# proroklab/gnn_pathplanning

Hardware: AMD Instinct MI355X
Metric: agent-steps/sec (policy fwd) (higher is better)
Workload: dtype f32 (bf16x3 exact operand split, f32 accumulate); 1 GPU; policy forward (addGSO+forward), 10 agents, 20x20 map GSO, K=3, batch=512 per GPU, eval mode, fp32 GSO resident in HBM; the SAME resident batch every step (inputs are L2 / Infinity-Cache warm by construction); agents=10, taps=3, batch_per_gpu=512, global_batch=512, parallelism=replicas x1

## Files before the change

### gnn_pathplanning_amd/csrc/encoder_kernel_b3.hip

```cpp
#include <utility>

#include "gnnpp_common.h"

namespace gnnpp {

constexpr int kb_L1 = 0, kb_L2 = 54, kb_L3 = 108, kb_L4 = 162, kb_FC = 270, kb_END = 294;
constexpr int kb_FILT = kb_END;

constexpr int kB3Frag = 1024;
constexpr int kB3Region = 25 * 3 * kB3Frag;
constexpr int kB3Obs2 = kObsFloatsLds * 4;
constexpr int kB3L2out = 0, kB3L3out = 24 * kB3Frag, kB3L4out = 48 * kB3Frag;
constexpr int kB3Table = kB3Region;
constexpr int kB3TableBytes = EncLayout::kBssFloats * 4 + 16;
constexpr int kB3TableBytesFused = 5120;
constexpr int kB3SsmOff = 776 * 4;
constexpr size_t kB3Smem = kB3Region + kB3TableBytes;
constexpr size_t kB3SmemFused = kB3Region + kB3TableBytesFused;
static_assert(2 * kObsFloatsLds * 4 <= kB3Region && kB3SsmOff + 16 * 17 * 4 <= kB3TableBytesFused &&
              2 * kB3SmemFused <= (size_t)kLdsBytes, "b3 LDS map");
constexpr int kB3ZBytes = 16 * kZs * 4;
constexpr int kB3PRow = 3 * 256 + 32;
constexpr int kB3PBytes = 16 * kB3PRow;
constexpr int kB3POff = 2 * kB3ZBytes;
static_assert(kB3POff + kPolicyTapsMax * kB3PBytes + 4 * 16 * 8 * 4 <= kB3Region, "fused tail fits R");
constexpr size_t policy_sim_occ_bytes_b3() {
    return (size_t)kB3POff - 8 * kMaxAgents * sizeof(int) - kGsoSmemBytes;
}

struct WStreamB {
    const float* seg[6];
    int lane_bytes;
};

__device__ __forceinline__ const float* ring_item_ptr(const WStreamB& ws, int idx) {
    if (idx < kb_L2) return ws.seg[0] + (idx - kb_L1) * EncLayout::kHItem;
    if (idx < kb_L3) return ws.seg[1] + (idx - kb_L2) * EncLayout::kHItem;
    if (idx < kb_L4) return ws.seg[2] + (idx - kb_L3) * EncLayout::kHItem;
    if (idx < kb_FC) return ws.seg[3] + (idx - kb_L4) * EncLayout::kHItem;
    if (idx < kb_FILT) return ws.seg[4] + (idx - kb_FC) * EncLayout::kHItem;
    const int j = idx - kb_FILT, pl = j % 3, ml = (j / 3) & 1, kb = (j / 6) & 3, tap = j / 24;
    return ws.seg[5] + tap * (8 * 4 * 768) + ml * (4 * 768) + kb * 768 + pl * 256;
}

template <int IT, int NKB, int H, int W, int NMT, int NSLOT, class PosFn, bool PRELOAD, int CH = NSLOT>
__device__ __forceinline__ void b3_tap_mfma(const v4f* in, const v4f* Pin, const v8b (&A)[NMT][3],
                                            v4f (&acc)[NSLOT][NMT], int lane) {
    constexpr int kb = IT / 9, tap = IT % 9;
    constexpr int dy = tap / 3 - 1, dx = tap % 3 - 1;
#pragma unroll
    for (int j0 = 0; j0 < NSLOT; j0 += CH) {
        v8b B[CH][3];
#pragma unroll
        for (int jj = 0; jj < CH; ++jj) {
            const int j = j0 + jj;
            int y = 0, x = 0;
            const bool used = j < NSLOT && PosFn::get(j, y, x);
            const int iy = y + dy, ix = x + dx;
            if (used && iy >= 0 && iy < H && ix >= 0 && ix < W) {
                const int o = ((iy * W + ix) * NKB + kb) * 3;
#pragma unroll
                for (int p = 0; p < 3; ++p) B[jj][p] = as_b8(PRELOAD ? Pin[o + p] : in[(o + p) * 64 + lane]);
            }
        }
#pragma unroll
        for (int term = 0; term < kB3Terms; ++term) {
#pragma unroll
            for (int jj = 0; jj < CH; ++jj) {
                const int j = j0 + jj;
                int y = 0, x = 0;
                const bool used = j < NSLOT && PosFn::get(j, y, x);
                const int iy = y + dy, ix = x + dx;
                if (used && iy >= 0 && iy < H && ix >= 0 && ix < W) {
// ... 210 lines not shown
            const int wy = win / 5, wx = win - wy * 5;
            const unsigned* base = obsw + (2 * wy) * kPadHW + 2 * wx;
            v4f acc[4][2];
#pragma unroll
            for (int pp = 0; pp < 4; ++pp) {
                unsigned d1[8], d2[8];
#pragma unroll
                for (int e = 0; e < 8; ++e) {
                    d1[e] = base[aoff[e] + (pp >> 1) * kPadHW + (pp & 1)];
                    d2[e] = base[kObsFloatsLds + aoff[e] + (pp >> 1) * kPadHW + (pp & 1)];
                }
                unsigned bh[4], bm[4], bl[4];
#pragma unroll
                for (int w = 0; w < 4; ++w) {
                    bh[w] = __builtin_amdgcn_perm(d1[2 * w + 1], d1[2 * w], 0x05040100u);
                    bm[w] = __builtin_amdgcn_perm(d1[2 * w + 1], d1[2 * w], 0x07060302u);
                    bl[w] = __builtin_amdgcn_perm(d2[2 * w + 1], d2[2 * w], 0x05040100u);
                }
                const v4u bhv = {bh[0], bh[1], bh[2], bh[3]}, bmv = {bm[0], bm[1], bm[2], bm[3]},
                          blv = {bl[0], bl[1], bl[2], bl[3]};
                const v8b B[3] = {__builtin_bit_cast(v8b, bhv), __builtin_bit_cast(v8b, bmv),
                                  __builtin_bit_cast(v8b, blv)};
#pragma unroll
                for (int term = 0; term < kB3Terms; ++term)
#pragma unroll
                    for (int i = 0; i < 2; ++i)
                        acc[pp][i] = mfma16b(A0[i][b3_term_a(term)], B[b3_term_b(term)],
                                             term == 0 ? vzero() : acc[pp][i]);
            }
#pragma unroll
            for (int i = 0; i < 2; ++i) {
                v4f sc, sh;
                load_ss(sstab + EncLayout::kBssL0, 32, i, q, sc, sh);
                v4f r = vmax(vmax(acc[0][i], acc[1][i]), vmax(acc[2][i], acc[3][i]));
                r = vfma(r, sc, sh);
#pragma unroll
                for (int c = 0; c < 4; ++c) r[c] = b3_relu_clamp(r[c]);
                res[wi][i] = r;
            }
        }
    }
    __syncthreads();
#pragma unroll
    for (int wi = 0; wi < 7; ++wi) {
        const int win = wave + 4 * wi;
        if (win < 25) {
            v4f pl[3];
            b3_split8_clamped(res[wi][0], res[wi][1], pl);
            b3_store_window<CP>(smem, g, win, lane, pl);
        }
    }
}

template <bool ONE_PLANE, bool CP>
__device__ __forceinline__ void b3_l0_stream(const float* __restrict__ pk, const unsigned* obsw,
                                             const float* sstab, char* smem, const CpGeom& g,
                                             v4f (&res)[ONE_PLANE ? 3 : 5][2], int wave, int lane) {
    constexpr int DEPTH = ONE_PLANE ? 3 : 1;
    constexpr int NHELD = ONE_PLANE ? 3 : 5;
    static_assert((4 * NHELD) * 3 * kB3Frag >= (ONE_PLANE ? 1 : 2) * kObsFloatsLds * 4, "held windows cover the pixels");
    constexpr int NW = ONE_PLANE ? 8 : 16;
    const int a = lane & 15, q = lane >> 4;
    v8b A0[2][3];
#pragma unroll
    for (int i = 0; i < 2; ++i)
#pragma unroll
        for (int p = 0; p < 3; ++p)
            A0[i][p] = as_b8(*reinterpret_cast<const v4f*>(pk + EncLayout::kB0 + ((i * 3 + p) * 64 + lane) * 4));
    int aoff[8];
#pragma unroll
    for (int e = 0; e < 8; ++e)
        aoff[e] = a * kAgentStride + (q < 3 ? q * (kPadHW * kPadHW) + (e / 3) * kPadHW + e % 3
                                            : e < 3 ? e * (kPadHW * kPadHW) + 2 * kPadHW + 2 : 0);
    v4f sc[2], sh[2];
    load_ss(sstab + EncLayout::kBssL0, 32, 0, q, sc[0], sh[0]);
    load_ss(sstab + EncLayout::kBssL0, 32, 1, q, sc[1], sh[1]);
    unsigned d[DEPTH + 1][NW];
    v4f acc[2][2];
    v4f run[2];
    auto request = [&](unsigned (&dd)[NW], int P) {
        const int win = wave + 4 * (P >> 2), pp = P & 3;
        const int wy = win / 5, wx = win - wy * 5;
        const unsigned* base = obsw + (2 * wy + (pp >> 1)) * kPadHW + 2 * wx + (pp & 1);
#pragma unroll
        for (int e = 0; e < 8; ++e) {
            dd[e] = base[aoff[e]];
            if (!ONE_PLANE) dd[8 + e] = base[kObsFloatsLds + aoff[e]];
        }
    };
    auto compute = [&](const unsigned (&dd)[NW], v4f (&ac)[2]) {
        unsigned bh[4], bm[4], bl[4];
#pragma unroll
        for (int w = 0; w < 4; ++w) {
            bh[w] = __builtin_amdgcn_perm(dd[2 * w + 1], dd[2 * w], 0x05040100u);
            if (!ONE_PLANE) {
                bm[w] = __builtin_amdgcn_perm(dd[2 * w + 1], dd[2 * w], 0x07060302u);
                bl[w] = __builtin_amdgcn_perm(dd[8 + 2 * w + 1], dd[8 + 2 * w], 0x05040100u);
            }
        }
        const v4u bhv = {bh[0], bh[1], bh[2], bh[3]};
        const v8b Bh = __builtin_bit_cast(v8b, bhv);
        if (ONE_PLANE) {
#pragma unroll
            for (int p = 2; p >= 0; --p)
#pragma unroll
                for (int i = 0; i < 2; ++i) ac[i] = mfma16b(A0[i][p], Bh, p == 2 ? vzero() : ac[i]);
        } else {
            const v4u bmv = {bm[0], bm[1], bm[2], bm[3]}, blv = {bl[0], bl[1], bl[2], bl[3]};
            const v8b B[3] = {Bh, __builtin_bit_cast(v8b, bmv), __builtin_bit_cast(v8b, blv)};
#pragma unroll
            for (int term = 0; term < kB3Terms; ++term)
#pragma unroll
                for (int i = 0; i < 2; ++i)
                    ac[i] = mfma16b(A0[i][b3_term_a(term)], B[b3_term_b(term)], term == 0 ? vzero() : ac[i]);
        }
    };
    auto epilogue = [&](const v4f (&ac)[2], int P) {
#pragma unroll
        for (int i = 0; i < 2; ++i) {
            run[i] = (P & 3) == 0 ? ac[i] : vmax(run[i], ac[i]);
            if ((P & 3) == 3) {
                run[i] = vfma(run[i], sc[i], sh[i]);
#pragma unroll
                for (int c = 0; c < 4; ++c) run[i][c] = b3_relu_clamp(run[i][c]);
            }
        }
#if defined(__HIP_DEVICE_COMPILE__)
        asm volatile("" : "+v"(run[0]), "+v"(run[1]));
#endif
    };
    auto window_done = [&](auto wic) {
        constexpr int wi = decltype(wic)::value;
        if constexpr (wi < NHELD) {
            res[wi][0] = run[0];
            res[wi][1] = run[1];
        } else {
            const int win = wave + 4 * wi;
            v4f pl[3];
            b3_split8_clamped(run[0], run[1], pl);
            b3_store_window<CP>(smem, g, win, lane, pl);
        }
    };
    auto prologue = [&](auto p0c, auto p1c, auto kc) {
        constexpr int P = decltype(p0c)::value + decltype(kc)::value;
        if constexpr (P < decltype(p1c)::value) request(d[P % (DEPTH + 1)], P);
    };
    auto body = [&](auto p0c, auto p1c, auto kc) {
        constexpr int P0 = decltype(p0c)::value, P1 = decltype(p1c)::value, P = P0 + decltype(kc)::value;
        if constexpr (P + DEPTH < P1) request(d[(P + DEPTH) % (DEPTH + 1)], P + DEPTH);
        __builtin_amdgcn_sched_barrier(0);
        compute(d[P % (DEPTH + 1)], acc[P & 1]);
        if constexpr (P > P0) {
            epilogue(acc[(P - 1) & 1], P - 1);
            if constexpr (((P - 1) & 3) == 3) window_done(std::integral_constant<int, ((P - 1) >> 2)>{});
        }
        __builtin_amdgcn_sched_barrier(0);
        if constexpr (P == P1 - 1) {
            epilogue(acc[P & 1], P);
            window_done(std::integral_constant<int, (P >> 2)>{});
        }
    };
    auto stream = [&](auto p0c, auto p1c) {
        constexpr int N = decltype(p1c)::value - decltype(p0c)::value;
        auto pro = [&](auto... ks) { (prologue(p0c, p1c, ks), ...); };
        auto run_all = [&](auto... ks) { (body(p0c, p1c, ks), ...); };
        [&]<int... K>(std::integer_sequence<int, K...>) { pro(std::integral_constant<int, K>{}...); }(
            std::make_integer_sequence<int, DEPTH>{});
        [&]<int... K>(std::integer_sequence<int, K...>) { run_all(std::integral_constant<int, K>{}...); }(
            std::make_integer_sequence<int, N>{});
    };
    stream(std::integral_constant<int, 0>{}, std::integral_constant<int, 24>{});
    if (wave == 0) stream(std::integral_constant<int, 24>{}, std::integral_constant<int, 28>{});
}

__host__ __device__ __forceinline__ constexpr int cp_ring_item_at(int NA, int i, int s) {
    int first = -1, cnt = 0;
    for (int k = 0; k < 6; ++k)
        if (k * NA / 6 == i) { if (first < 0) first = k; ++cnt; }
    if (cnt == 0 || s % (6 / cnt) != 0 || s / (6 / cnt) >= cnt) return -1;
    return first + s / (6 / cnt);
}
template <class Load, class Hook>
__device__ __forceinline__ void cp_unit(const v8b (&A)[2][3], const v4f (&B)[3], v4f& c0, v4f& c1, Load&& load, Hook&& hook) {
#define GNNPP_CP_M(T, ACC, MI)                                                                          \
    ACC = mfma16b(A[MI][b3_term_a(T)], as_b8(B[b3_term_b(T)]), ACC);                                   \
    __builtin_amdgcn_sched_barrier(0);
#define GNNPP_CP_H(S)                                                                                   \
    hook(std::integral_constant<int, S>{});                                                             \
    __builtin_amdgcn_sched_barrier(0);
    GNNPP_CP_M(0, c0, 0)
    load(0);
    __builtin_amdgcn_sched_barrier(0);
    GNNPP_CP_M(0, c1, 1)
    load(1);
    __builtin_amdgcn_sched_barrier(0);
    GNNPP_CP_M(1, c0, 0)
    load(2);
    __builtin_amdgcn_sched_barrier(0);
    GNNPP_CP_M(1, c1, 1)
    GNNPP_CP_H(0)
    GNNPP_CP_M(2, c0, 0)
    GNNPP_CP_H(1)
    GNNPP_CP_M(2, c1, 1)
    GNNPP_CP_H(2)
// ... 289 lines not shown
        case 2: cp_layer2_main<END, 2>(ws, ring, smem, ln, pair, acc); break;
        case 3: cp_layer2_main<END, 3>(ws, ring, smem, ln, pair, acc); break;
        case 4: cp_layer2_main<END, 4>(ws, ring, smem, ln, pair, acc); break;
        case 5: cp_layer2_main<END, 5>(ws, ring, smem, ln, pair, acc); break;
        default: cp_layer2_main<END, 6>(ws, ring, smem, ln, pair, acc); break;
    }
    v4f sc[2], shf[2];
    load_ss(sstab + EncLayout::kBssL2, 64, 2 * mp, q, sc[0], shf[0]);
    load_ss(sstab + EncLayout::kBssL2, 64, 2 * mp + 1, q, sc[1], shf[1]);
    const bool hi2 = (p & 2) != 0, hi1 = (p & 1) != 0;
    float pooled[NT][2];
#pragma unroll
    for (int i = 0; i < NT; ++i) {
        pooled[i][0] = pooled[i][1] = 0.f;
        if (i < na) {
            const v4f v0 = vfma(acc[i][0], sc[0], shf[0]), v1 = vfma(acc[i][1], sc[1], shf[1]);
            v4f keep, send;
#pragma unroll
            for (int c = 0; c < 4; ++c) {
                keep[c] = hi2 ? v1[c] : v0[c];
                send[c] = hi2 ? v0[c] : v1[c];
            }
#pragma unroll
            for (int c = 0; c < 4; ++c) keep[c] = fmaxf(keep[c], quad_xor2(send[c]));
            const float k0 = hi1 ? keep[2] : keep[0], k1 = hi1 ? keep[3] : keep[1];
            const float s0 = hi1 ? keep[0] : keep[2], s1 = hi1 ? keep[1] : keep[3];
            pooled[i][0] = fmaxf(fmaxf(k0, quad_xor1(s0)), 0.f);
            pooled[i][1] = fmaxf(fmaxf(k1, quad_xor1(s1)), 0.f);
        }
    }
    __syncthreads();
#pragma unroll
    for (int i = 0; i < NT; ++i) {
        if (i < na) {
            const int n = pair + 2 * i;
            unsigned h, m, l;
            b3_split2(pooled[i][0], pooled[i][1], h, m, l);
            char* const dst = smem + kB3L2out + ((w * 2 + mp) * 3) * kB3Frag + (q * 16 + n) * 16 + p * 4;
            *reinterpret_cast<unsigned*>(dst) = h;
            *reinterpret_cast<unsigned*>(dst + kB3Frag) = m;
            *reinterpret_cast<unsigned*>(dst + 2 * kB3Frag) = l;
        }
    }
    if (j >= g.N) {
#pragma unroll
        for (int k = 0; k < 6; ++k)
            *reinterpret_cast<v4f*>(smem + kB3L2out + (wave + 4 * k) * kB3Frag + lane * 16) = vzero();
    }
}

template <bool FUSED, int KT, bool CP = false>
__global__ GNNPP_H2_VGPR_BUDGET __launch_bounds__(kThreads, 2) void encoder_kernel_b3(const float* __restrict__ obs,
                                                                 const float* __restrict__ pk,
                                                                 float* __restrict__ feat, int M, int stop,
                                                                 const PolicyTail pt) {
    constexpr int END = FUSED ? kb_FILT + 24 * KT : kb_END;
    extern __shared__ __attribute__((aligned(16))) char gnnpp_smem[];
    v4f* const R4 = reinterpret_cast<v4f*>(gnnpp_smem);
    unsigned* const obsw = reinterpret_cast<unsigned*>(gnnpp_smem);
    float* const sstab = reinterpret_cast<float*>(gnnpp_smem + kB3Table);
    unsigned* const planeflag = reinterpret_cast<unsigned*>(gnnpp_smem + kB3Table + EncLayout::kBssFloats * 4);
    const int tid = threadIdx.x;
    const int lane = tid & 63;
    const int wave = __builtin_amdgcn_readfirstlane(tid >> 6);
    const int a = lane & 15;
    const int q = lane >> 4;
    const int tile_agents = (FUSED || CP) ? pt.N : kTileAgents;
    const int agent0 = blockIdx.x * tile_agents;
    const int n_agents = FUSED ? pt.N : min(tile_agents, M - agent0);
    const CpGeom geom = cp_geom(CP ? n_agents : kTileAgents);
    GNNPP_STAMP(blockIdx.x, 11, tid == 0);

    WStreamB ws;
    ws.seg[0] = pk + EncLayout::kB1;
    ws.seg[1] = pk + EncLayout::kB2 + (wave & 1) * (54 * EncLayout::kHItem);
    ws.seg[2] = pk + EncLayout::kB3 + wave * (54 * EncLayout::kHItem);
    ws.seg[3] = pk + EncLayout::kB4 + wave * (108 * EncLayout::kHItem);
    ws.seg[4] = pk + EncLayout::kBfcw + wave * (24 * EncLayout::kHItem);
    ws.seg[5] = FUSED ? pt.filt_h2 + wave * (2 * 4 * 768) : pk;
    ws.lane_bytes = lane * 16;
    float ssv[3];
#pragma unroll
    for (int i = 0; i < 3; ++i)
        ssv[i] = pk[EncLayout::kBss + min(tid + i * kThreads, EncLayout::kBssFloats - 1)];
    float hcv[4] = {0.f, 0.f, 0.f, 0.f};
    float sval = 0.f;
    if (FUSED) {
#pragma unroll
        for (int i = 0; i < 4; ++i) {
            const int c = tid + i * kThreads;
            if (c < 640) hcv[i] = pt.act_w[c];
            else if (c < 768) hcv[i] = pt.gf_bias ? pt.gf_bias[c - 640] : 0.f;
            else if (c < 773) hcv[i] = pt.act_b[c - 768];
        }
        const int m = tid >> 4, n = tid & 15;
        if (m < pt.N && n < pt.N) {
            const size_t i = ((size_t)blockIdx.x * pt.N + m) * pt.N + n;
            sval = pt.s_is_f64 ? (float)reinterpret_cast<const double*>(pt.S)[i]
                               : reinterpret_cast<const float*>(pt.S)[i];
        }
    }
    v4f ring[kRingH];
#if defined(__HIP_DEVICE_COMPILE__)
    asm volatile("; weight ring lives in v[208:255]" ::: "v255");
#endif
#pragma unroll
    for (int i = 0; i < kRingH; ++i) h2_ring_load<END>(ws, ring, i);

    {
        constexpr int NV4 = (kTileAgents * kObsFloats + 3) / 4 + 1;
        constexpr int PER = (NV4 + kThreads - 1) / kThreads;
        const int valid = n_agents * kObsFloats;
        const float* src = obs + (size_t)agent0 * kObsFloats;
        const int shift = (int)((reinterpret_cast<uintptr_t>(src) >> 2) & 3);
        const float* src4 = src - shift;
        const long floats_left = (long)(M - agent0) * kObsFloats + shift;
        const bool head_ok = shift == 0 || agent0 > 0;
        v4f v[PER];
#pragma unroll
        for (int k = 0; k < PER; ++k) {
            const int idx = tid + k * kThreads;
            const int e0 = 4 * idx - shift;
            if (head_ok && 4L * idx + 4 <= floats_left && e0 < valid) {
                v[k] = *reinterpret_cast<const v4f*>(src4 + 4 * idx);
            } else {
#pragma unroll
                for (int c = 0; c < 4; ++c) v[k][c] = src[min(max(e0 + c, 0), valid - 1)];
            }
        }
        for (int i = tid; i < 2 * kObsFloatsLds / 4; i += kThreads) R4[i] = vzero();
        if (CP && tid < kCpRow / 16)
            *reinterpret_cast<v4f*>(gnnpp_smem + geom.l1in + geom.T1 * kCpRow + tid * 16) = vzero();
        unsigned residual = 0;
#pragma unroll
        for (int i = 0; i < 3; ++i)
            if (tid + i * kThreads < EncLayout::kBssFloats) sstab[tid + i * kThreads] = ssv[i];
        __syncthreads();
        const unsigned dump = 2 * kObsFloatsLds + lane;
#pragma unroll
        for (int k = 0; k < PER; ++k) {
            const int e0 = (tid + k * kThreads) * 4 - shift;
            const unsigned es = (unsigned)max(e0, 0);
            const unsigned ag = __umul24(es, 46223u) >> 24;
            const unsigned rem = es - __umul24(ag, (unsigned)kObsFloats);
            const unsigned ch = __umul24(rem, 543u) >> 16;
            const int r0 = (int)(rem - __umul24(ch, 121u)) + min(e0, 0);
            const unsigned base = __umul24(ag, (unsigned)kAgentStride) + __umul24(ch, (unsigned)(kPadHW * kPadHW)) + 13u;
            const unsigned wrapped = base + (ch == 2u ? (unsigned)(kAgentStride - 2 * kPadHW * kPadHW) : (unsigned)(kPadHW * kPadHW));
            unsigned w1[4], w2[4];
            const v4u vb = __builtin_bit_cast(v4u, v[k]);
            const bool inexact = ((vb[0] | vb[1] | vb[2] | vb[3]) & 0xffffu) != 0u;
            const bool any_l = __ballot(inexact) != 0ull;
            if (!any_l) {
                w1[0] = vb[0] >> 16; w1[1] = vb[1] >> 16; w1[2] = vb[2] >> 16; w1[3] = vb[3] >> 16;
            } else {
#pragma unroll
                for (int c2 = 0; c2 < 2; ++c2) {
                    unsigned h, m, l;
                    b3_split2(v[k][2 * c2], v[k][2 * c2 + 1], h, m, l);
                    residual |= m | l;
                    w1[2 * c2] = __builtin_amdgcn_perm(m, h, 0x05040100u);
                    w1[2 * c2 + 1] = __builtin_amdgcn_perm(m, h, 0x07060302u);
                    w2[2 * c2] = l & 0xffffu;
                    w2[2 * c2 + 1] = l >> 16;
                }
            }
#pragma unroll
            for (int c = 0; c < 4; ++c) {
                const int e = e0 + c;
                int r = r0 + c;
                const bool wrap = r >= 121;
                r = wrap ? r - 121 : r;
                const unsigned y = __umul24((unsigned)r & 0xffu, 745u) >> 13;
                const unsigned o = (wrap ? wrapped : base) + (unsigned)r + y;
                const bool ok = e >= 0 && e < valid;
                obsw[ok ? o : dump] = w1[c];
                if (any_l) obsw[ok ? o + kObsFloatsLds : dump] = w2[c];
            }
        }
        const bool wave_residual = __ballot(residual != 0) != 0ull;
        if (lane == 0) planeflag[wave] = wave_residual ? 1u : 0u;
    }
    __syncthreads();
    if (GNNPP_STOP_AT(stop, 1)) return;
    if (!pt.with_sim) GNNPP_STAMP(blockIdx.x, 0, tid == 0);

    {
        const v4u pf = *reinterpret_cast<const v4u*>(planeflag);
        const bool one_plane = (pf[0] | pf[1] | pf[2] | pf[3]) == 0;
        if (one_plane) {
            v4f res[3][2];
            b3_l0_stream<true, CP>(pk, obsw, sstab, gnnpp_smem, geom, res, wave, lane);
            __syncthreads();
#pragma unroll
            for (int wi = 0; wi < 3; ++wi) {
                const int win = wave + 4 * wi;
                v4f pl[3];
                b3_split8_clamped(res[wi][0], res[wi][1], pl);
                b3_store_window<CP>(gnnpp_smem, geom, win, lane, pl);
            }
        } else {
            b3_l0_generic<CP>(pk, obsw, sstab, gnnpp_smem, geom, wave, lane);
        }
    }
    __syncthreads();
    if (GNNPP_STOP_AT(stop, 2)) return;
    if (!pt.with_sim) GNNPP_STAMP(blockIdx.x, 1, tid == 0);

    if constexpr (CP) {
        cp_layer1<END>(ws, ring, gnnpp_smem, sstab, geom, wave, lane, tid);
    } else {
        v4f acc[7][2];
        constexpr int CH1 = 2;
        v4f Bb[2][CH1][3];
        auto layer1 = [&](auto wc) {
            using P = PosL1H<decltype(wc)::value>;
            b3_load_chunk<0, 0, 1, 5, 5, 7, CH1, P>(R4, Bb[0], lane);
            b3_stream_steps<END, kb_L1, 2>(ws, ring, [&](auto itc, const v8b (&A)[2][3]) {
                b3_step_pipelined<decltype(itc)::value, 9, 1, 5, 5, 2, 7, CH1, P>(R4, Bb, A, acc, lane);
            }, std::make_integer_sequence<int, 9>{});
        };
        switch (wave) {
            case 0: layer1(std::integral_constant<int, 0>{}); break;
            case 1: layer1(std::integral_constant<int, 1>{}); break;
            case 2: layer1(std::integral_constant<int, 2>{}); break;
            default: layer1(std::integral_constant<int, 3>{}); break;
        }
        __syncthreads();
        v4f sc[2], sh[2];
        load_ss(sstab + EncLayout::kBssL1, 32, 0, q, sc[0], sh[0]);
        load_ss(sstab + EncLayout::kBssL1, 32, 1, q, sc[1], sh[1]);
#pragma unroll
        for (int j = 0; j < 7; ++j) {
            const int p = wave + 4 * j;
            if (p < 25) {
                v4f pl[3];
                b3_split8_clamped(vrelu_clamp(vfma(acc[j][0], sc[0], sh[0])), vrelu_clamp(vfma(acc[j][1], sc[1], sh[1])), pl);
#pragma unroll
                for (int pp = 0; pp < 3; ++pp) R4[(p * 3 + pp) * 64 + lane] = pl[pp];
            }
        }
    }
    __syncthreads();
    if (GNNPP_STOP_AT(stop, 3)) return;
    if (!pt.with_sim) GNNPP_STAMP(blockIdx.x, 2, tid == 0);

    if constexpr (CP) {
        cp_layer2<END>(ws, ring, gnnpp_smem, sstab, geom, wave, lane);
// ... 209 lines not shown
    float* const yb = reinterpret_cast<float*>(gnnpp_smem + kB3POff + KT * kB3PBytes);
    {
        v4f d = vzero();
#pragma unroll
        for (int m = 0; m < 2; ++m) {
            const int f0 = (2 * wave + m) * 16 + 4 * q;
            const v4f bv = *reinterpret_cast<const v4f*>(hconst + 640 + f0);
            const v4f A5 = a < 5 ? *reinterpret_cast<const v4f*>(hconst + a * 128 + f0) : vzero();
            d = mfma16x4(A5, vrelu((fa[m] + fc[m]) + bv), d);
        }
        if (q < 2) *reinterpret_cast<v4f*>(yb + (wave * 16 + a) * 8 + 4 * q) = d;
    }
    __syncthreads();
    int* const spos = reinterpret_cast<int*>(gnnpp_smem);
    if (wave == 0) {
        v4f d = *reinterpret_cast<const v4f*>(yb + a * 8 + 4 * (q & 1));
#pragma unroll
        for (int w = 1; w < kWaves; ++w) d += *reinterpret_cast<const v4f*>(yb + (w * 16 + a) * 8 + 4 * (q & 1));
        const v4f ab4 = *reinterpret_cast<const v4f*>(hconst + 768 + 4 * (q & 1));
        if (a < pt.N && q < 2) {
            float* dst = pt.logits + ((size_t)a * pt.B + blockIdx.x) * 5;
            float* lds = reinterpret_cast<float*>(spos) + 4 * kMaxAgents + a * 5;
            if (q == 0) {
#pragma unroll
                for (int t = 0; t < 4; ++t) {
                    dst[t] = d[t] + ab4[t];
                    if (pt.with_sim) lds[t] = d[t] + ab4[t];
                }
            } else {
                dst[4] = d[0] + ab4[0];
                if (pt.with_sim) lds[4] = d[0] + ab4[0];
            }
        }
        __builtin_amdgcn_wave_barrier();
    }
    if (!pt.with_sim) return;

    {
        int* red = spos + 2 * kMaxAgents;
        int* goal_l = red + 4 * kMaxAgents;
        char* gso_smem = reinterpret_cast<char*>(goal_l + 2 * kMaxAgents);
        unsigned char* occ = reinterpret_cast<unsigned char*>(gso_smem + kGsoSmemBytes);
        const int b = blockIdx.x;
        GNNPP_STAMP(b, 10, tid == 0);
        const size_t occ_bytes = ((size_t)pt.sim.H * pt.sim.W + 15) & ~(size_t)15;
        unsigned* cellcnt = 2 * occ_bytes <= policy_sim_occ_bytes_b3() ? reinterpret_cast<unsigned*>(occ + occ_bytes)
                                                                       : nullptr;
        sim_tail(pt.sim, b, spos, red, goal_l, gso_smem, occ, tid, kThreads, cellcnt,
                 reinterpret_cast<const float*>(red + 2 * kMaxAgents));
    }
}

std::atomic<int> g_policy_column_packing{1};
std::atomic<int> g_encoder_cp_tile{0};

static int encoder_cp_tile(int M) {
    const int knob = g_encoder_cp_tile.load(std::memory_order_relaxed);
    if (knob >= 1 && knob <= kCpMaxAgents) return knob;
    if (knob != 0 || g_policy_column_packing.load(std::memory_order_relaxed) == 0) return 0;
    const int t = (M + 255) / 256;
    return t <= 8 ? t : 0;
}

int encoder_launch_b3(const float* obs, const float* packed, float* feat, int M, hipStream_t st) {
    if (const int tile = encoder_cp_tile(M)) {
        static LdsAttrOnce once_cp;
        set_lds_attr_once(once_cp, reinterpret_cast<const void*>(&encoder_kernel_b3<false, 3, true>), (int)kB3Smem);
        PolicyTail pt{};
        pt.N = tile;
        hipLaunchKernelGGL((encoder_kernel_b3<false, 3, true>), dim3((M + tile - 1) / tile), dim3(kThreads), kB3Smem, st,
                           obs, packed, feat, M, GNNPP_ENCODER_STOP_VALUE, pt);
        return hipGetLastError() == hipSuccess ? 0 : -3;
    }
    static LdsAttrOnce once;
    set_lds_attr_once(once, reinterpret_cast<const void*>(&encoder_kernel_b3<false, 3>), (int)kB3Smem);
    const int grid = (M + kTileAgents - 1) / kTileAgents;
    hipLaunchKernelGGL((encoder_kernel_b3<false, 3>), dim3(grid), dim3(kThreads), kB3Smem, st, obs, packed, feat, M,
                       GNNPP_ENCODER_STOP_VALUE, PolicyTail{});
    return hipGetLastError() == hipSuccess ? 0 : -3;
}

template <int KT, bool CP>
static int policy_launch_fused_b3_k(const float* obs, const float* packed, const PolicyTail& pt, hipStream_t st) {
    static LdsAttrOnce once;
    set_lds_attr_once(once, reinterpret_cast<const void*>(&encoder_kernel_b3<true, KT, CP>), (int)kB3SmemFused);
    hipLaunchKernelGGL((encoder_kernel_b3<true, KT, CP>), dim3(pt.B), dim3(kThreads), kB3SmemFused, st, obs, packed,
                       static_cast<float*>(nullptr), pt.B * pt.N, 0, pt);
    return hipGetLastError() == hipSuccess ? 0 : -3;
}

int policy_launch_fused_b3(const float* obs, const float* packed, const PolicyTail& pt, int K, hipStream_t st) {
    const bool cp = pt.N <= kCpMaxAgents && g_policy_column_packing.load(std::memory_order_relaxed) != 0;
    switch (K) {
        case 2: return cp ? policy_launch_fused_b3_k<2, true>(obs, packed, pt, st)
                          : policy_launch_fused_b3_k<2, false>(obs, packed, pt, st);
        case 3: return cp ? policy_launch_fused_b3_k<3, true>(obs, packed, pt, st)
                          : policy_launch_fused_b3_k<3, false>(obs, packed, pt, st);
        case 4: return cp ? policy_launch_fused_b3_k<4, true>(obs, packed, pt, st)
                          : policy_launch_fused_b3_k<4, false>(obs, packed, pt, st);
        default: return -2;
    }
}

}
```

### gnn_pathplanning_amd/csrc/gnnpp_api.hip

```cpp
#include "../../include/gnnpp.h"
#ifdef GNNPP_MEASURE
#include "gnnpp_measure.h"
#endif

#include "encoder_pack.hip"
#include "encoder_ring_f32.hip"
#include "encoder_kernel_f32.hip"
#include "rollout_kernels.hip"
#include "rollout_team_kernels.hip"
#include "expert_kernels.hip"
#include "expert_team_kernels.hip"
#include "mapf_kernels.hip"
#include "mapf_team_kernels.hip"
#include "encoder_kernel_h2.hip"
#include "encoder_kernel_b3.hip"
#include "lsigf_kernel.hip"
#include "policy_filter_kernel.hip"
#include "lsigf_small_kernel.hip"
#include "lsigf_team_kernel.hip"
#include "train_encoder.hip"
#include "train_ops.hip"

using namespace gnnpp;

// ... 378 lines not shown
int gnnpp_policy_loss(const float* logits, const float* target, float* loss, float* dlogits, int B, int N,
                      int C, int logits_sample_major, void* stream) {
    if (!logits || !target || !loss || B <= 0 || N <= 0 || C <= 0 || C > 64) return GNNPP_ERR_ARG;
    hipLaunchKernelGGL(policy_loss_kernel, dim3(1), dim3(1024), 1024 * sizeof(double),
                       static_cast<hipStream_t>(stream), logits, target, loss, dlogits, B, N, C, logits_sample_major);
    return hipGetLastError() == hipSuccess ? GNNPP_OK : GNNPP_ERR_LAUNCH;
}

int gnnpp_adam_step(const gnnpp_adam_tensors* t, float* state, float lr, float beta1, float beta2, float eps,
                    float weight_decay, int tick, void* stream) {
    if (!t || !state || t->count <= 0 || t->count > kAdamTensors) return GNNPP_ERR_ARG;
    hipStream_t st = static_cast<hipStream_t>(stream);
    AdamTable tb = {};
    int blocks = 0;
    for (int i = 0; i < t->count; ++i) {
        if (!t->p[i] || !t->g[i] || !t->m[i] || !t->v[i] || t->numel[i] <= 0) return GNNPP_ERR_ARG;
        tb.p[i] = t->p[i]; tb.g[i] = t->g[i]; tb.m[i] = t->m[i]; tb.v[i] = t->v[i];
        tb.numel[i] = (long)t->numel[i];
        tb.first[i] = blocks;
        blocks += (int)((t->numel[i] + 1023) / 1024);
    }
    tb.first[t->count] = blocks;
    tb.count = t->count;
    hipLaunchKernelGGL(adam_kernel, dim3(blocks), dim3(256), 4 * sizeof(float), st, tb, state, lr, beta1, beta2, eps,
                       weight_decay, tick ? 1 : 0);
    return hipGetLastError() == hipSuccess ? GNNPP_OK : GNNPP_ERR_LAUNCH;
}

#ifdef GNNPP_MEASURE
int gnnpp_measure_read_stamps(unsigned long long* host, int n) {
    if (!host || n <= 0 || n > 1024 * 32) return GNNPP_ERR_ARG;
    return hipMemcpyFromSymbol(host, HIP_SYMBOL(g_stamps), (size_t)n * sizeof(unsigned long long)) == hipSuccess
               ? GNNPP_OK : GNNPP_ERR_LAUNCH;
}
#endif

int gnnpp_get_tuning(int key) {
    switch (key) {
        case GNNPP_TUNE_FILTER_GPW: return g_filter_gpw.load();
        case GNNPP_TUNE_FILTER_WAVES: return g_filter_waves.load();
        case GNNPP_TUNE_FUSED_POLICY: return g_fused_policy.load();
        case GNNPP_TUNE_FILTER_SPLIT: return g_filter_split.load();
        case GNNPP_TUNE_POLICY_FILTER: return g_filter_policy_kernel.load();
        case GNNPP_TUNE_FILTER_SMALL: return g_filter_small_kernel.load();
        case GNNPP_TUNE_FILTER_SMALL_ROWS: return g_filter_small_rows.load();
        case GNNPP_TUNE_FILTER_PIPE_GRID: return g_filter_pipe_grid.load();
        case GNNPP_TUNE_POLICY_CP: return g_policy_column_packing.load();
        case GNNPP_TUNE_ENCODER_CP_TILE: return g_encoder_cp_tile.load();
        case GNNPP_TUNE_TRAIN_FORK: return g_train_fork.load();
        case GNNPP_TUNE_FILTER_PLANE_ALIAS: return g_filter_plane_alias.load();
        case GNNPP_TUNE_TRAIN_WGRAD_WGS: return g_train_wgrad_wgs.load();
        case GNNPP_TUNE_TRAIN_WGRAD_MERGED: return g_train_wgrad_merged.load();
        case GNNPP_TUNE_TRAIN_RUNNING_FUSED: return g_train_running_fused.load();
#ifdef GNNPP_MEASURE
        case GNNPP_TUNE_FILTER_ABLATE: return g_filter_ablate.load();
        case GNNPP_TUNE_ENCODER_STOP: return g_encoder_stop.load();
#endif
        default: return GNNPP_ERR_ARG;
    }
}

int gnnpp_set_tuning(int key, int value) {
    switch (key) {
        case GNNPP_TUNE_FILTER_GPW:
            if (value < 0) return GNNPP_ERR_ARG;
            g_filter_gpw.store(value);
            return GNNPP_OK;
        case GNNPP_TUNE_FUSED_POLICY:
            if (value < 0 || value > 2) return GNNPP_ERR_ARG;
            g_fused_policy.store(value);
            return GNNPP_OK;
        case GNNPP_TUNE_FILTER_WAVES:
            if (value != 0 && value != 8 && value != 16) return GNNPP_ERR_ARG;
            g_filter_waves.store(value);
            return GNNPP_OK;
        case GNNPP_TUNE_FILTER_SPLIT:
            if (value < 0 || value > 7) return GNNPP_ERR_ARG;
            g_filter_split.store(value);
            return GNNPP_OK;
        case GNNPP_TUNE_POLICY_FILTER:
            if (value < 0 || value > 1) return GNNPP_ERR_ARG;
            g_filter_policy_kernel.store(value);
            return GNNPP_OK;
        case GNNPP_TUNE_FILTER_SMALL_ROWS:
            if (value != 0 && value != 32 && value != 48 && value != 64) return GNNPP_ERR_ARG;
            g_filter_small_rows.store(value);
            return GNNPP_OK;
        case GNNPP_TUNE_FILTER_PIPE_GRID:
            if (value < 0 || value > 4096) return GNNPP_ERR_ARG;
            g_filter_pipe_grid.store(value);
            return GNNPP_OK;
        case GNNPP_TUNE_POLICY_CP:
            if (value != 0 && value != 1) return GNNPP_ERR_ARG;
            g_policy_column_packing.store(value);
            return GNNPP_OK;
        case GNNPP_TUNE_ENCODER_CP_TILE:
            if (value != 0 && value != 16 && (value < 1 || value > 12)) return GNNPP_ERR_ARG;
            g_encoder_cp_tile.store(value);
            return GNNPP_OK;
        case GNNPP_TUNE_TRAIN_FORK:
            if (value < 0 || value > 2) return GNNPP_ERR_ARG;
            g_train_fork.store(value);
            return GNNPP_OK;
        case GNNPP_TUNE_FILTER_PLANE_ALIAS:
            if (value < 0 || value > 1) return GNNPP_ERR_ARG;
            g_filter_plane_alias.store(value);
            return GNNPP_OK;
        case GNNPP_TUNE_TRAIN_WGRAD_MERGED:
            if (value < 0 || value > 1) return GNNPP_ERR_ARG;
            g_train_wgrad_merged.store(value);
            return GNNPP_OK;
        case GNNPP_TUNE_TRAIN_RUNNING_FUSED:
            if (value < 0 || value > 1) return GNNPP_ERR_ARG;
            g_train_running_fused.store(value);
            return GNNPP_OK;
        case GNNPP_TUNE_TRAIN_WGRAD_WGS:
            if (value != 0 && (value < 16 || value > 2048)) return GNNPP_ERR_ARG;
            g_train_wgrad_wgs.store(value);
            return GNNPP_OK;
        case GNNPP_TUNE_FILTER_SMALL:
            if (value < 0 || value > 3) return GNNPP_ERR_ARG;
            g_filter_small_kernel.store(value);
            return GNNPP_OK;
#ifdef GNNPP_MEASURE
        case GNNPP_TUNE_ENCODER_STOP:
            if (value < 0 || value > 6) return GNNPP_ERR_ARG;
            g_encoder_stop.store(value);
            return GNNPP_OK;
        case GNNPP_TUNE_FILTER_ABLATE:
            g_filter_ablate.store(value);
            return GNNPP_OK;
#endif
        default:
            return GNNPP_ERR_ARG;
    }
}

int gnnpp_decode_actions(const float* logits, int* actions, int B, int N, void* stream) {
    if (!logits || !actions || B <= 0 || N <= 0) return GNNPP_ERR_ARG;
    return decode_actions_launch(logits, actions, B, N, static_cast<hipStream_t>(stream));
}

static int rollout_common_ok(const gnnpp_rollout* r, int max_agents = GNNPP_ROLLOUT_MAX_TEAM) {
    return r && r->pos && r->B > 0 && r->N > 0 && r->N <= max_agents;
}

static bool rollout_team(const gnnpp_rollout* r) { return r->N > GNNPP_ROLLOUT_MAX_AGENTS; }

int gnnpp_rollout_observe(const gnnpp_rollout* r, void* stream) {
    if (!rollout_common_ok(r) || !r->grid || !r->goal || !r->obs || r->H <= 0 || r->W <= 0)
        return GNNPP_ERR_ARG;
    if (rollout_team(r)) return rollout_team_observe_launch(*r, static_cast<hipStream_t>(stream));
    return rollout_observe_launch(*r, static_cast<hipStream_t>(stream));
}

int gnnpp_rollout_gso(const gnnpp_rollout* r, void* stream) {
    if (!rollout_common_ok(r) || !r->radius || !r->S) return GNNPP_ERR_ARG;
    if (rollout_team(r)) return rollout_team_gso_launch(*r, r->grow != 0, static_cast<hipStream_t>(stream));
    return rollout_gso_launch(*r, static_cast<hipStream_t>(stream));
}

int gnnpp_rollout_gso_observe(const gnnpp_rollout* r, void* stream) {
    if (!rollout_common_ok(r) || !r->radius || !r->S || !r->grid || !r->goal || !r->obs || r->H <= 0 || r->W <= 0)
        return GNNPP_ERR_ARG;
    if (rollout_team(r)) return rollout_team_gso_observe_launch(*r, static_cast<hipStream_t>(stream));
    return rollout_gso_observe_launch(*r, static_cast<hipStream_t>(stream));
}
// ... 133 lines not shown
```

### include/gnnpp.h

```cpp
#ifndef GNNPP_H_
#define GNNPP_H_

#include <stddef.h>

#ifdef __cplusplus
extern "C" {
#endif

#define GNNPP_OK               0
#define GNNPP_ERR_ARG         (-1)
#define GNNPP_ERR_UNSUPPORTED (-2)
#define GNNPP_ERR_LAUNCH      (-3)
#define GNNPP_ERR_RANGE       (-4)

#define GNNPP_PREC_FP32        0
#define GNNPP_PREC_FP32_MFMA   1
#define GNNPP_PREC_SPLIT_F16   2

#define GNNPP_OBS_C        3
#define GNNPP_OBS_HW       11
#define GNNPP_FEAT         128
#define GNNPP_ACTIONS      5
#define GNNPP_MAX_NODES    100
#define GNNPP_MAX_ROWS     112

int         gnnpp_version(void);
const char* gnnpp_error_string(int code);

#define GNNPP_TUNE_FILTER_GPW      1
#define GNNPP_TUNE_FILTER_WAVES    2
#define GNNPP_TUNE_FILTER_SPLIT    7
#define GNNPP_TUNE_FUSED_POLICY     6
#define GNNPP_TUNE_POLICY_FILTER    9
#define GNNPP_TUNE_FILTER_SMALL     10
#define GNNPP_TUNE_FILTER_SMALL_ROWS 11
#define GNNPP_TUNE_FILTER_PIPE_GRID 12
#define GNNPP_TUNE_POLICY_CP        13
#define GNNPP_TUNE_ENCODER_CP_TILE   14
#define GNNPP_TUNE_TRAIN_FORK        15
#define GNNPP_TUNE_FILTER_PLANE_ALIAS 16
#define GNNPP_TUNE_TRAIN_WGRAD_WGS   17
#define GNNPP_TUNE_TRAIN_WGRAD_MERGED 18
#define GNNPP_TUNE_TRAIN_RUNNING_FUSED 19
int         gnnpp_set_tuning(int key, int value);
int         gnnpp_get_tuning(int key);


size_t gnnpp_filter_packed_floats(int G, int F, int K, int E);

int gnnpp_filter_pack(const float* h, float* packed, int G, int F, int K, int E, void* stream);

int gnnpp_lsigf_fwd(const float* x, const void* S, const float* packed, const float* bias,
                    float* y, int B, int N, int Nin, int G, int F, int K, int E,
                    int s_is_f64, int s_batched, int x_node_major, int y_node_major, int relu,
                    int bias_per_node, int precision, int* range_flag, void* stream);


int gnnpp_lsigf_fwd_save(const float* x, const void* S, const float* packed, const float* bias,
                         float* y, float* zs, int B, int N, int Nin, int G, int F, int K, int E,
                         int s_is_f64, int s_batched, int s_transposed, int x_node_major,
                         int y_node_major, int relu, int bias_per_node, int precision, int* range_flag,
                         void* stream);

int gnnpp_lsigf_fits(int N, int G, int F, int K, int E);


typedef struct gnnpp_encoder_params {
    const float* conv_w[5];
    const float* conv_b[5];
    const float* bn_w[5];
    const float* bn_b[5];
    const float* bn_mean[5];
    const float* bn_var[5];
    const float* fc_w;
    const float* fc_b;
    float        bn_eps;
} gnnpp_encoder_params;

size_t gnnpp_encoder_packed_floats(void);

int gnnpp_encoder_pack(const gnnpp_encoder_params* params, float* packed, void* stream);

int gnnpp_encoder_fwd(const float* obs, const float* packed, float* feat, int M, int precision,
                      int* range_flag, void* stream);

typedef struct gnnpp_encoder_grads {
    float* conv_w[5];
    float* conv_b[5];
    float* bn_w[5];
    float* bn_b[5];
} gnnpp_encoder_grads;

size_t gnnpp_encoder_train_workspace_floats(int N, int B);
int gnnpp_encoder_train_fwd(const gnnpp_encoder_params* p, const float* obs, float* workspace, float* feat,
                            int B, int N, float momentum, int update_running,
                            long long* const* bn_num_batches, int feat_sample_major, const float* train_pack,
// ... 186 lines not shown
```

Measured before the change: 98.66 million agent-steps/s.

## Pack exact-bf16 observation pixels as 16-bit halves for the one-plane L0 stream

The kernel now decides, before the scatter, whether every loaded observation value is exactly representable in bf16. In that case it scatters pixels as 16-bit halves into a compact per-agent/channel image and zeroes only that smaller region. The one-plane L0 convolution stream is rewritten to read 7 packed words per pair of horizontal sub-positions and assemble MFMA operands with per-lane perm selectors, with deeper prefetch and fewer held windows. The intent is to cut LDS footprint, LDS load count and zero-fill work in the common binary-map case. In exchange the code adds a ballot, an extra sync on the multi-plane fallback, a host tuning flag to force planes, and new tight static_asserts on the layout.

New measurement: 101.2 million agent-steps/s (median of 6 runs). +2.5%, better.

```diff
diff --git a/gnn_pathplanning_amd/csrc/encoder_kernel_b3.hip b/gnn_pathplanning_amd/csrc/encoder_kernel_b3.hip
--- a/gnn_pathplanning_amd/csrc/encoder_kernel_b3.hip
+++ b/gnn_pathplanning_amd/csrc/encoder_kernel_b3.hip
@@ -19,6 +19,13 @@
 constexpr size_t kB3SmemFused = kB3Region + kB3TableBytesFused;
 static_assert(2 * kObsFloatsLds * 4 <= kB3Region && kB3SsmOff + 16 * 17 * 4 <= kB3TableBytesFused &&
               2 * kB3SmemFused <= (size_t)kLdsBytes, "b3 LDS map");
+constexpr int kPkChan = 73;
+constexpr int kPkAgent = 231;
+constexpr int kPkBytes = kTileAgents * kPkAgent * 4;
+constexpr int kB3ForcePlanes = 256;
+constexpr int kL0Held = 2;
+static_assert(kPkChan >= kPadHW * kPadHW / 2 && kPkAgent >= 3 * kPkChan && (kPkAgent & 1) && kPkBytes % 16 == 0 &&
+              kPkBytes <= 2 * kObsFloatsLds * 4, "packed pixel image");
 constexpr int kB3ZBytes = 16 * kZs * 4;
 constexpr int kB3PRow = 3 * 256 + 32;
 constexpr int kB3PBytes = 16 * kB3PRow;
@@ -335,14 +342,22 @@
     }
 }
 
-template <bool ONE_PLANE, bool CP>
+__host__ __device__ constexpr bool cp_direct_windows_clear_pixels() {
+    for (int N = 1; N <= kCpMaxAgents; ++N) {
+        const int T1 = (25 * N + 15) >> 4, l1in = kB3Region - (T1 + 1) * kCpRow;
+        if (l1in + ((4 * kL0Held * N) >> 4) * kCpRow < kPkBytes) return false;
+    }
+    return true;
+}
+
+template <bool CP>
 __device__ __forceinline__ void b3_l0_stream(const float* __restrict__ pk, const unsigned* obsw,
                                              const float* sstab, char* smem, const CpGeom& g,
-                                             v4f (&res)[ONE_PLANE ? 3 : 5][2], int wave, int lane) {
-    constexpr int DEPTH = ONE_PLANE ? 3 : 1;
-    constexpr int NHELD = ONE_PLANE ? 3 : 5;
-    static_assert((4 * NHELD) * 3 * kB3Frag >= (ONE_PLANE ? 1 : 2) * kObsFloatsLds * 4, "held windows cover the pixels");
-    constexpr int NW = ONE_PLANE ? 8 : 16;
+                                             v4f (&res)[kL0Held][2], int wave, int lane) {
+    constexpr int DEPTH = 2;
+    constexpr int NHELD = kL0Held;
+    static_assert((4 * NHELD) * 3 * kB3Frag >= kPkBytes, "held windows cover the pixels");
+    static_assert(!CP || cp_direct_windows_clear_pixels(), "column-packed windows written early lie behind the pixels");
     const int a = lane & 15, q = lane >> 4;
     v8b A0[2][3];
 #pragma unroll
@@ -350,53 +365,50 @@
 #pragma unroll
         for (int p = 0; p < 3; ++p)
             A0[i][p] = as_b8(*reinterpret_cast<const v4f*>(pk + EncLayout::kB0 + ((i * 3 + p) * 64 + lane) * 4));
-    int aoff[8];
-#pragma unroll
-    for (int e = 0; e < 8; ++e)
-        aoff[e] = a * kAgentStride + (q < 3 ? q * (kPadHW * kPadHW) + (e / 3) * kPadHW + e % 3
-                                            : e < 3 ? e * (kPadHW * kPadHW) + 2 * kPadHW + 2 : 0);
+    const int ab = a * kPkAgent, pb = ab + q * kPkChan;
+    int adr[5];
+    adr[0] = q < 3 ? pb : ab + 13;
+    adr[1] = q < 3 ? pb + 1 : ab + kPkChan + 13;
+    adr[2] = q < 3 ? pb + 1 : ab + 2 * kPkChan + 13;
+    adr[3] = q < 3 ? pb + 6 : ab;
+    adr[4] = q < 3 ? pb + 12 : ab;
+    unsigned selA[2], selC[2], selD[2];
+    selA[0] = q < 3 ? 0x03020100u : 0x05040100u;  selA[1] = q < 3 ? 0x05040302u : 0x07060302u;
+    selC[0] = q < 3 ? 0x05040302u : 0x01000100u;  selC[1] = q < 3 ? 0x07060504u : 0x03020302u;
+    selD[0] = q < 3 ? 0x03020100u : 0x01000100u;  selD[1] = q < 3 ? 0x05040302u : 0x03020302u;
+#if defined(__HIP_DEVICE_COMPILE__)
+    asm volatile("" : "+v"(adr[0]), "+v"(adr[1]), "+v"(adr[2]), "+v"(adr[3]), "+v"(adr[4]));
+    asm volatile("" : "+v"(selA[0]), "+v"(selA[1]), "+v"(selC[0]), "+v"(selC[1]), "+v"(selD[0]), "+v"(selD[1]));
+#endif
     v4f sc[2], sh[2];
     load_ss(sstab + EncLayout::kBssL0, 32, 0, q, sc[0], sh[0]);
     load_ss(sstab + EncLayout::kBssL0, 32, 1, q, sc[1], sh[1]);
-    unsigned d[DEPTH + 1][NW];
+    unsigned d[DEPTH + 1][7];
     v4f acc[2][2];
     v4f run[2];
-    auto request = [&](unsigned (&dd)[NW], int P) {
-        const int win = wave + 4 * (P >> 2), pp = P & 3;
+    auto request = [&](unsigned (&dd)[7], int H) {
+        const int win = wave + 4 * (H >> 1);
         const int wy = win / 5, wx = win - wy * 5;
-        const unsigned* base = obsw + (2 * wy + (pp >> 1)) * kPadHW + 2 * wx + (pp & 1);
-#pragma unroll
-        for (int e = 0; e < 8; ++e) {
-            dd[e] = base[aoff[e]];
-            if (!ONE_PLANE) dd[8 + e] = base[kObsFloatsLds + aoff[e]];
-        }
+        const unsigned* base = obsw + (2 * wy + (H & 1)) * (kPadHW / 2) + wx;
+        dd[0] = base[adr[0]];
+        dd[4] = base[adr[0] + 7];
+        dd[1] = base[adr[1]];
+        dd[2] = base[adr[2]];
+        dd[3] = base[adr[3]];
+        dd[5] = base[adr[4]];
+        dd[6] = base[adr[4] + 1];
     };
-    auto compute = [&](const unsigned (&dd)[NW], v4f (&ac)[2]) {
-        unsigned bh[4], bm[4], bl[4];
-#pragma unroll
-        for (int w = 0; w < 4; ++w) {
-            bh[w] = __builtin_amdgcn_perm(dd[2 * w + 1], dd[2 * w], 0x05040100u);
-            if (!ONE_PLANE) {
-                bm[w] = __builtin_amdgcn_perm(dd[2 * w + 1], dd[2 * w], 0x07060302u);
-                bl[w] = __builtin_amdgcn_perm(dd[8 + 2 * w + 1], dd[8 + 2 * w], 0x05040100u);
-            }
-        }
-        const v4u bhv = {bh[0], bh[1], bh[2], bh[3]};
+    auto compute = [&](const unsigned (&dd)[7], auto oxc, v4f (&ac)[2]) {
+        constexpr int ox = decltype(oxc)::value;
+        const v4u bhv = {__builtin_amdgcn_perm(dd[1], dd[0], selA[ox]),
+                         __builtin_amdgcn_perm(dd[3], dd[2], ox ? 0x07060302u : 0x05040100u),
+                         __builtin_amdgcn_perm(dd[4], dd[3], selC[ox]),
+                         __builtin_amdgcn_perm(dd[6], dd[5], selD[ox])};
         const v8b Bh = __builtin_bit_cast(v8b, bhv);
-        if (ONE_PLANE) {
-#pragma unroll
-            for (int p = 2; p >= 0; --p)
-#pragma unroll
-                for (int i = 0; i < 2; ++i) ac[i] = mfma16b(A0[i][p], Bh, p == 2 ? vzero() : ac[i]);
-        } else {
-            const v4u bmv = {bm[0], bm[1], bm[2], bm[3]}, blv = {bl[0], bl[1], bl[2], bl[3]};
-            const v8b B[3] = {Bh, __builtin_bit_cast(v8b, bmv), __builtin_bit_cast(v8b, blv)};
-#pragma unroll
-            for (int term = 0; term < kB3Terms; ++term)
-#pragma unroll
-                for (int i = 0; i < 2; ++i)
-                    ac[i] = mfma16b(A0[i][b3_term_a(term)], B[b3_term_b(term)], term == 0 ? vzero() : ac[i]);
-        }
+#pragma unroll
+        for (int p = 2; p >= 0; --p)
+#pragma unroll
+            for (int i = 0; i < 2; ++i) ac[i] = mfma16b(A0[i][p], Bh, p == 2 ? vzero() : ac[i]);
     };
     auto epilogue = [&](const v4f (&ac)[2], int P) {
 #pragma unroll
@@ -425,14 +437,14 @@
         }
     };
     auto prologue = [&](auto p0c, auto p1c, auto kc) {
-        constexpr int P = decltype(p0c)::value + decltype(kc)::value;
-        if constexpr (P < decltype(p1c)::value) request(d[P % (DEPTH + 1)], P);
+        constexpr int H = decltype(p0c)::value / 2 + decltype(kc)::value;
+        if constexpr (H < decltype(p1c)::value / 2) request(d[H % (DEPTH + 1)], H);
     };
     auto body = [&](auto p0c, auto p1c, auto kc) {
-        constexpr int P0 = decltype(p0c)::value, P1 = decltype(p1c)::value, P = P0 + decltype(kc)::value;
-        if constexpr (P + DEPTH < P1) request(d[(P + DEPTH) % (DEPTH + 1)], P + DEPTH);
+        constexpr int P0 = decltype(p0c)::value, P1 = decltype(p1c)::value, P = P0 + decltype(kc)::value, H = P >> 1;
+        if constexpr ((P & 1) == 0 && H + DEPTH < P1 / 2) request(d[(H + DEPTH) % (DEPTH + 1)], H + DEPTH);
         __builtin_amdgcn_sched_barrier(0);
-        compute(d[P % (DEPTH + 1)], acc[P & 1]);
+        compute(d[H % (DEPTH + 1)], std::integral_constant<int, (P & 1)>{}, acc[P & 1]);
         if constexpr (P > P0) {
             epilogue(acc[(P - 1) & 1], P - 1);
             if constexpr (((P - 1) & 3) == 3) window_done(std::integral_constant<int, ((P - 1) >> 2)>{});
@@ -828,9 +840,11 @@
 template <bool FUSED, int KT, bool CP = false>
 __global__ GNNPP_H2_VGPR_BUDGET __launch_bounds__(kThreads, 2) void encoder_kernel_b3(const float* __restrict__ obs,
                                                                  const float* __restrict__ pk,
-                                                                 float* __restrict__ feat, int M, int stop,
+                                                                 float* __restrict__ feat, int M, int stop_flags,
                                                                  const PolicyTail pt) {
     constexpr int END = FUSED ? kb_FILT + 24 * KT : kb_END;
+    [[maybe_unused]] const int stop = stop_flags & 255;
+    const bool force_planes = (stop_flags & kB3ForcePlanes) != 0;
     extern __shared__ __attribute__((aligned(16))) char gnnpp_smem[];
     v4f* const R4 = reinterpret_cast<v4f*>(gnnpp_smem);
     unsigned* const obsw = reinterpret_cast<unsigned*>(gnnpp_smem);
@@ -883,6 +897,7 @@
 #pragma unroll
     for (int i = 0; i < kRingH; ++i) h2_ring_load<END>(ws, ring, i);
 
+    bool one_plane;
     {
         constexpr int NV4 = (kTileAgents * kObsFloats + 3) / 4 + 1;
         constexpr int PER = (NV4 + kThreads - 1) / kThreads;
@@ -904,72 +919,94 @@
                 for (int c = 0; c < 4; ++c) v[k][c] = src[min(max(e0 + c, 0), valid - 1)];
             }
         }
-        for (int i = tid; i < 2 * kObsFloatsLds / 4; i += kThreads) R4[i] = vzero();
+        unsigned lowbits = 0;
+#pragma unroll
+        for (int k = 0; k < PER; ++k) {
+            const v4u vb = __builtin_bit_cast(v4u, v[k]);
+            lowbits |= vb[0] | vb[1] | vb[2] | vb[3];
+        }
+        const bool wave_inexact = __ballot((lowbits & 0xffffu) != 0u) != 0ull;
+        if (lane == 0) planeflag[wave] = (wave_inexact || force_planes) ? 1u : 0u;
+        for (int i = tid; i < kPkBytes / 16; i += kThreads) R4[i] = vzero();
         if (CP && tid < kCpRow / 16)
             *reinterpret_cast<v4f*>(gnnpp_smem + geom.l1in + geom.T1 * kCpRow + tid * 16) = vzero();
-        unsigned residual = 0;
 #pragma unroll
         for (int i = 0; i < 3; ++i)
             if (tid + i * kThreads < EncLayout::kBssFloats) sstab[tid + i * kThreads] = ssv[i];
         __syncthreads();
+        {
+            const v4u pf = *reinterpret_cast<const v4u*>(planeflag);
+            one_plane = __builtin_amdgcn_readfirstlane((int)(pf[0] | pf[1] | pf[2] | pf[3])) == 0;
+        }
         const unsigned dump = 2 * kObsFloatsLds + lane;
-#pragma unroll
-        for (int k = 0; k < PER; ++k) {
-            const int e0 = (tid + k * kThreads) * 4 - shift;
-            const unsigned es = (unsigned)max(e0, 0);
-            const unsigned ag = __umul24(es, 46223u) >> 24;
-            const unsigned rem = es - __umul24(ag, (unsigned)kObsFloats);
-            const unsigned ch = __umul24(rem, 543u) >> 16;
-            const int r0 = (int)(rem - __umul24(ch, 121u)) + min(e0, 0);
-            const unsigned base = __umul24(ag, (unsigned)kAgentStride) + __umul24(ch, (unsigned)(kPadHW * kPadHW)) + 13u;
-            const unsigned wrapped = base + (ch == 2u ? (unsigned)(kAgentStride - 2 * kPadHW * kPadHW) : (unsigned)(kPadHW * kPadHW));
-            unsigned w1[4], w2[4];
-            const v4u vb = __builtin_bit_cast(v4u, v[k]);
-            const bool inexact = ((vb[0] | vb[1] | vb[2] | vb[3]) & 0xffffu) != 0u;
-            const bool any_l = __ballot(inexact) != 0ull;
-            if (!any_l) {
-                w1[0] = vb[0] >> 16; w1[1] = vb[1] >> 16; w1[2] = vb[2] >> 16; w1[3] = vb[3] >> 16;
-            } else {
-#pragma unroll
-                for (int c2 = 0; c2 < 2; ++c2) {
-                    unsigned h, m, l;
-                    b3_split2(v[k][2 * c2], v[k][2 * c2 + 1], h, m, l);
-                    residual |= m | l;
-                    w1[2 * c2] = __builtin_amdgcn_perm(m, h, 0x05040100u);
-                    w1[2 * c2 + 1] = __builtin_amdgcn_perm(m, h, 0x07060302u);
-                    w2[2 * c2] = l & 0xffffu;
-                    w2[2 * c2 + 1] = l >> 16;
+        auto scatter = [&](auto packedc) {
+            constexpr bool PACKED = decltype(packedc)::value;
+            constexpr unsigned AS = PACKED ? 2 * kPkAgent : kAgentStride, CS = PACKED ? 2 * kPkChan : kPadHW * kPadHW;
+            unsigned short* const obsh = reinterpret_cast<unsigned short*>(gnnpp_smem);
+#pragma unroll
+            for (int k = 0; k < PER; ++k) {
+                const int e0 = (tid + k * kThreads) * 4 - shift;
+                const unsigned es = (unsigned)max(e0, 0);
+                const unsigned ag = __umul24(es, 46223u) >> 24;
+                const unsigned rem = es - __umul24(ag, (unsigned)kObsFloats);
+                const unsigned ch = __umul24(rem, 543u) >> 16;
+                const int r0 = (int)(rem - __umul24(ch, 121u)) + min(e0, 0);
+                const unsigned base = __umul24(ag, AS) + __umul24(ch, CS) + 13u;
+                const unsigned wrapped = base + (ch == 2u ? AS - 2 * CS : CS);
+                unsigned w1[4], w2[4];
+                const v4u vb = __builtin_bit_cast(v4u, v[k]);
+                const bool inexact = ((vb[0] | vb[1] | vb[2] | vb[3]) & 0xffffu) != 0u;
+                const bool any_l = !PACKED && __ballot(inexact) != 0ull;
+                if (!any_l) {
+                    w1[0] = vb[0] >> 16; w1[1] = vb[1] >> 16; w1[2] = vb[2] >> 16; w1[3] = vb[3] >> 16;
+                } else {
+#pragma unroll
+                    for (int c2 = 0; c2 < 2; ++c2) {
+                        unsigned h, m, l;
+                        b3_split2(v[k][2 * c2], v[k][2 * c2 + 1], h, m, l);
+                        w1[2 * c2] = __builtin_amdgcn_perm(m, h, 0x05040100u);
+                        w1[2 * c2 + 1] = __builtin_amdgcn_perm(m, h, 0x07060302u);
+                        w2[2 * c2] = l & 0xffffu;
+                        w2[2 * c2 + 1] = l >> 16;
+                    }
                 }
-            }
-#pragma unroll
-            for (int c = 0; c < 4; ++c) {
-                const int e = e0 + c;
-                int r = r0 + c;
-                const bool wrap = r >= 121;
-                r = wrap ? r - 121 : r;
-                const unsigned y = __umul24((unsigned)r & 0xffu, 745u) >> 13;
-                const unsigned o = (wrap ? wrapped : base) + (unsigned)r + y;
-                const bool ok = e >= 0 && e < valid;
-                obsw[ok ? o : dump] = w1[c];
-                if (any_l) obsw[ok ? o + kObsFloatsLds : dump] = w2[c];
-            }
-        }
-        const bool wave_residual = __ballot(residual != 0) != 0ull;
-        if (lane == 0) planeflag[wave] = wave_residual ? 1u : 0u;
+#pragma unroll
+                for (int c = 0; c < 4; ++c) {
+                    const int e = e0 + c;
+                    int r = r0 + c;
+                    const bool wrap = r >= 121;
+                    r = wrap ? r - 121 : r;
+                    const unsigned y = __umul24((unsigned)r & 0xffu, 745u) >> 13;
+                    const unsigned o = (wrap ? wrapped : base) + (unsigned)r + y;
+                    const bool ok = e >= 0 && e < valid;
+                    if constexpr (PACKED) {
+                        obsh[ok ? o : 2 * dump] = (unsigned short)w1[c];
+                    } else {
+                        obsw[ok ? o : dump] = w1[c];
+                        if (any_l) obsw[ok ? o + kObsFloatsLds : dump] = w2[c];
+                    }
+                }
+            }
+        };
+        if (one_plane) {
+            scatter(std::true_type{});
+        } else {
+            for (int i = kPkBytes / 16 + tid; i < 2 * kObsFloatsLds / 4; i += kThreads) R4[i] = vzero();
+            __syncthreads();
+            scatter(std::false_type{});
+        }
     }
     __syncthreads();
     if (GNNPP_STOP_AT(stop, 1)) return;
     if (!pt.with_sim) GNNPP_STAMP(blockIdx.x, 0, tid == 0);
 
     {
-        const v4u pf = *reinterpret_cast<const v4u*>(planeflag);
-        const bool one_plane = (pf[0] | pf[1] | pf[2] | pf[3]) == 0;
         if (one_plane) {
-            v4f res[3][2];
-            b3_l0_stream<true, CP>(pk, obsw, sstab, gnnpp_smem, geom, res, wave, lane);
+            v4f res[kL0Held][2];
+            b3_l0_stream<CP>(pk, obsw, sstab, gnnpp_smem, geom, res, wave, lane);
             __syncthreads();
 #pragma unroll
-            for (int wi = 0; wi < 3; ++wi) {
+            for (int wi = 0; wi < kL0Held; ++wi) {
                 const int win = wave + 4 * wi;
                 v4f pl[3];
                 b3_split8_clamped(res[wi][0], res[wi][1], pl);
@@ -1285,6 +1322,8 @@
 }
 
 std::atomic<int> g_policy_column_packing{1};
+std::atomic<int> g_encoder_one_plane{1};
+static int b3_plane_flag() { return g_encoder_one_plane.load(std::memory_order_relaxed) ? 0 : kB3ForcePlanes; }
 std::atomic<int> g_encoder_cp_tile{0};
 
 static int encoder_cp_tile(int M) {
@@ -1302,14 +1341,14 @@
         PolicyTail pt{};
         pt.N = tile;
         hipLaunchKernelGGL((encoder_kernel_b3<false, 3, true>), dim3((M + tile - 1) / tile), dim3(kThreads), kB3Smem, st,
-                           obs, packed, feat, M, GNNPP_ENCODER_STOP_VALUE, pt);
+                           obs, packed, feat, M, GNNPP_ENCODER_STOP_VALUE | b3_plane_flag(), pt);
         return hipGetLastError() == hipSuccess ? 0 : -3;
     }
     static LdsAttrOnce once;
     set_lds_attr_once(once, reinterpret_cast<const void*>(&encoder_kernel_b3<false, 3>), (int)kB3Smem);
     const int grid = (M + kTileAgents - 1) / kTileAgents;
     hipLaunchKernelGGL((encoder_kernel_b3<false, 3>), dim3(grid), dim3(kThreads), kB3Smem, st, obs, packed, feat, M,
-                       GNNPP_ENCODER_STOP_VALUE, PolicyTail{});
+                       GNNPP_ENCODER_STOP_VALUE | b3_plane_flag(), PolicyTail{});
     return hipGetLastError() == hipSuccess ? 0 : -3;
 }
 
@@ -1318,7 +1357,7 @@
     static LdsAttrOnce once;
     set_lds_attr_once(once, reinterpret_cast<const void*>(&encoder_kernel_b3<true, KT, CP>), (int)kB3SmemFused);
     hipLaunchKernelGGL((encoder_kernel_b3<true, KT, CP>), dim3(pt.B), dim3(kThreads), kB3SmemFused, st, obs, packed,
-                       static_cast<float*>(nullptr), pt.B * pt.N, 0, pt);
+                       static_cast<float*>(nullptr), pt.B * pt.N, b3_plane_flag(), pt);
     return hipGetLastError() == hipSuccess ? 0 : -3;
 }
 
diff --git a/gnn_pathplanning_amd/csrc/gnnpp_api.hip b/gnn_pathplanning_amd/csrc/gnnpp_api.hip
--- a/gnn_pathplanning_amd/csrc/gnnpp_api.hip
+++ b/gnn_pathplanning_amd/csrc/gnnpp_api.hip
@@ -454,6 +454,7 @@
         case GNNPP_TUNE_TRAIN_WGRAD_WGS: return g_train_wgrad_wgs.load();
         case GNNPP_TUNE_TRAIN_WGRAD_MERGED: return g_train_wgrad_merged.load();
         case GNNPP_TUNE_TRAIN_RUNNING_FUSED: return g_train_running_fused.load();
+        case GNNPP_TUNE_ENCODER_ONE_PLANE: return g_encoder_one_plane.load();
 #ifdef GNNPP_MEASURE
         case GNNPP_TUNE_FILTER_ABLATE: return g_filter_ablate.load();
         case GNNPP_TUNE_ENCODER_STOP: return g_encoder_stop.load();
@@ -515,6 +516,10 @@
         case GNNPP_TUNE_TRAIN_RUNNING_FUSED:
             if (value < 0 || value > 1) return GNNPP_ERR_ARG;
             g_train_running_fused.store(value);
+            return GNNPP_OK;
+        case GNNPP_TUNE_ENCODER_ONE_PLANE:
+            if (value < 0 || value > 1) return GNNPP_ERR_ARG;
+            g_encoder_one_plane.store(value);
             return GNNPP_OK;
         case GNNPP_TUNE_TRAIN_WGRAD_WGS:
             if (value != 0 && (value < 16 || value > 2048)) return GNNPP_ERR_ARG;
diff --git a/include/gnnpp.h b/include/gnnpp.h
--- a/include/gnnpp.h
+++ b/include/gnnpp.h
@@ -42,6 +42,7 @@
 #define GNNPP_TUNE_TRAIN_WGRAD_WGS   17
 #define GNNPP_TUNE_TRAIN_WGRAD_MERGED 18
 #define GNNPP_TUNE_TRAIN_RUNNING_FUSED 19
+#define GNNPP_TUNE_ENCODER_ONE_PLANE 20
 int         gnnpp_set_tuning(int key, int value);
 int         gnnpp_get_tuning(int key);
 
```
